# QData/FastSK

Measured on AMD Instinct MI355X. Metric: gkm kernel build: mismatch-combos/s, higher is better.
Workload: dtype u4 count planes (v_dot8_u32_u4), u32 register sums, u64 triangle (plain stores on the first pass over reset rows, else atomics); 1 GPU; config5: synthetic DNA 100000 x 300 bp, g=12 m=8 exact, 495 combos; n_seq=100000, seq_len=300, g=12, m=8, combos=495, parallelism=single GPU

## Files before the change

fastsk_amd/csrc/fsk_engine_dense_shift.hip:

```cpp
#include "fsk_engine_internal.h"
#include "fsk_kernels_dense_shift.h"

#include <map>

using namespace fsk_detail;

namespace fsk {

#define FSK_DMA_SHIFT 1
#define FSK_DMA_KERNEL k_dense_tile_shift
#define FSK_DMA_COMPACT 0
#include "fsk_tile_kernel_dma.inc"
#undef FSK_DMA_KERNEL
#undef FSK_DMA_SHIFT

#define FSK_DMA_SHIFT 2
#define FSK_DMA_KERNEL k_dense_tile_shift_all
#include "fsk_tile_kernel_dma.inc"
#undef FSK_DMA_KERNEL
#undef FSK_DMA_COMPACT
#undef FSK_DMA_SHIFT

}

namespace fsk_detail {

bool dense_shift_plan(fsk_engine* e, const int32_t* combos, int n, u64 by_overflow, uint32_t max_chain) {
    ShiftPlan& p = e->shift;
    if (!(p.by_overflow == by_overflow && p.max_chain == max_chain && (int)p.combos.size() == n && std::equal(combos, combos + n, p.combos.begin()))) {
        p = ShiftPlan();
        p.combos.assign(combos, combos + n);
        p.by_overflow = by_overflow;
        p.max_chain = max_chain;
        const int k = e->k;
        std::map<std::vector<uint8_t>, std::vector<std::pair<int, int>>> shapes;
        for (int q = 0; q < n; ++q) {
            const uint8_t* pos = &e->all_pos[(size_t)combos[q] * k];
            std::vector<uint8_t> shape(pos, pos + k);
            for (auto& x : shape) x = (uint8_t)(x - pos[0]);
            shapes[shape].push_back({(int)pos[0], q});
        }
        std::vector<std::vector<int>> chains;
        for (auto& kv : shapes) {
            auto& v = kv.second;
            std::stable_sort(v.begin(), v.end(), [](const std::pair<int, int>& a, const std::pair<int, int>& b) { return a.first < b.first; });
            for (size_t i = 0; i < v.size(); ++i) {
                if (i == 0 || v[i].first != v[i - 1].first + 1 || (max_chain != 0u && chains.back().size() >= max_chain)) chains.emplace_back();
                chains.back().push_back(v[i].second);
            }
        }
        std::stable_sort(chains.begin(), chains.end(), [](const std::vector<int>& a, const std::vector<int>& b) { return a.size() > b.size(); });
        p.n_bases = (uint32_t)chains.size();
        p.order.resize((size_t)n);
        uint32_t derived = p.n_bases;
        size_t group_begin = 0;
        for (size_t c = 0; c < chains.size(); ++c) {
            const std::vector<int>& ch = chains[c];
            const uint32_t len = (uint32_t)ch.size();
            p.order[c] = ch[0];
            if (c == 0 || chains[c - 1].size() != ch.size() || (u64)(c - group_begin) >= by_overflow) {
                p.groups.push_back(0u);
                p.groups.push_back(len);
                group_begin = c;
            }
            p.groups[p.groups.size() - 2] = (uint32_t)c + 1u;
            uint32_t lower = (uint32_t)c;
            for (uint32_t u = 1; u < len; ++u) {
                const uint32_t upper = derived++;
                p.order[upper] = ch[u];
                p.steps.push_back(upper << 16 | lower);
                p.steps.push_back(len - u);
                p.wsum += len - u;
                lower = upper;
            }
        }
        bool falling = true;
        for (size_t gi = 2; gi + 1 < p.groups.size(); gi += 2) falling = falling && p.groups[gi + 1] < p.groups[gi - 1];
        if (falling) {
            for (size_t gi = 0; gi + 1 < p.groups.size(); gi += 2) {
                p.group_steps.push_back(p.groups[gi]);
                p.group_steps.push_back(p.groups[gi + 1] - (gi + 3 < p.groups.size() ? p.groups[gi + 3] : 0u));
            }
            p.group_steps.push_back(0xffffffffu);
            p.group_steps.push_back(0u);
        }
    }
    return !p.steps.empty() && n <= 32768 && ((u64)2 * e->maxW + 32) * p.wsum < ((u64)1 << 31);
}

int dense_shift_edge_keys(fsk_engine* e, const uint8_t* chunk_pos, uint32_t panels_pad) {
    ShiftPlan& p = e->shift;
    const uint32_t n_steps = (uint32_t)(p.steps.size() / 2), np_seq = panels_pad * fsk::PANEL;
    FSK_HIP(e->d_shift_steps.reserve(p.steps.size() + p.group_steps.size()));
    FSK_HIP(e->d_edge_keys.reserve((size_t)n_steps * np_seq));
    FSK_HIP(hipMemcpyAsync(e->d_shift_steps.p, p.steps.data(), p.steps.size() * sizeof(uint32_t), hipMemcpyHostToDevice, e->stream));
    if (!p.group_steps.empty())
        FSK_HIP(hipMemcpyAsync(e->d_shift_steps.p + p.steps.size(), p.group_steps.data(), p.group_steps.size() * sizeof(uint32_t), hipMemcpyHostToDevice,
                               e->stream));
    FSK_LAUNCH(fsk::k_dense_edge_keys, dim3(panels_pad, (n_steps + 3u) / 4u), dim3(256), 0, e->stream, e->view(), e->cfg.g, e->k, e->sigma, chunk_pos,
               (const uint32_t*)e->d_shift_steps.p, n_steps, np_seq, e->d_edge_keys.p);
    FSK_HIP(hipStreamSynchronize(e->stream));
    e->st.launches += 1;
    return FSK_OK;
}

int dense_shift_keymajor(fsk_engine* e, uint32_t panels_pad, int nb, uint32_t Vq8) {
    const ShiftPlan& p = e->shift;
    e->ld.shift_packed = false;
    if (e->tune.dense_shift_packed < 0 || p.max_chain != SHIFT_PACKED_CHAIN) return FSK_OK;
    const size_t plane = (size_t)panels_pad * Vq8 * fsk::PANEL * (size_t)nb;
    const size_t n_keys = (p.steps.size() / 2) * (size_t)panels_pad * fsk::PANEL;
    const size_t want = (2 * plane + n_keys) * sizeof(uint32_t);
    const char* why = nullptr;
    if (e->tune.dense_shift_plane_kb > 0 && want > (size_t)e->tune.dense_shift_plane_kb * 1024) why = "over the dense_shift_plane_kb cap";
    const size_t grow = (std::max(plane, e->d_KM.cap) - e->d_KM.cap + std::max(plane, e->d_KMH.cap) - e->d_KMH.cap +
                         std::max(n_keys, e->d_edge_offs.cap) - e->d_edge_offs.cap) * sizeof(uint32_t);
    if (!why && grow > 0) {
        size_t free_b = 0, total_b = 0;
        if (hipMemGetInfo(&free_b, &total_b) != hipSuccess) free_b = 0;
        if (grow > free_b / 2) why = "more than half of the free device memory";
        else if (e->d_KM.reserve(plane) != hipSuccess || e->d_KMH.reserve(plane) != hipSuccess || e->d_edge_offs.reserve(n_keys) != hipSuccess) {
            (void)hipGetLastError();
            e->d_KM.release(); e->d_KMH.release(); e->d_edge_offs.release();
            why = "hipMalloc failed";
        }
    }
    if (why) {
        if (e->trace())
            fprintf(stderr, "[fsk] dense shift classes: the key-major planes (%.1f MB) do not fit, %s: k_dense_shift_fix runs the corrections\n",
                    (double)want / 1e6, why);
        return FSK_OK;
    }
    const uint32_t n_pairs = panels_pad / 2u;
    const uint32_t kgrid = (uint32_t)(((size_t)n_pairs * nb * Vq8 * 16u + 255u) / 256u);
    FSK_LAUNCH(fsk::k_dense_keymajor, dim3(kgrid), dim3(256), 0, e->stream, (const uint32_t*)e->d_C4.p, n_pairs, nb, Vq8, e->d_KM.p);
    FSK_LAUNCH(fsk::k_dense_keymajor, dim3(kgrid), dim3(256), 0, e->stream, (const uint32_t*)e->d_C4H.p, n_pairs, nb, Vq8, e->d_KMH.p);
    FSK_LAUNCH(fsk::k_dense_edge_offs, dim3((uint32_t)((n_keys + 255u) / 256u)), dim3(256), 0, e->stream, (const uint16_t*)e->d_edge_keys.p, n_keys,
               e->d_edge_offs.p);
    e->st.launches += 3;
    e->ld.shift_packed = true;
    return FSK_OK;
}

int dense_shift_tiles(fsk_engine* e, u64 n_tiles, int nb, uint32_t Vq8, uint32_t nst, u64* K, int store, uint32_t panels_pad) {
    const ShiftPlan& p = e->shift;
    const bool one_launch = !p.group_steps.empty() && (e->tune.dense_shift_one_launch > 0 ||
                                                       (e->tune.dense_shift_one_launch == 0 && e->tune.tile_splits == 0 && n_tiles >= 16384));
    int base_launches = 1;
    if (one_launch) {
        FSK_LAUNCH(fsk::k_dense_tile_shift_all, dim3((uint32_t)n_tiles, 1), dim3(256), 0, e->stream, (const uint32_t*)e->d_C4.p,
                   (const uint32_t*)e->d_C4H.p, (const uint32_t*)e->d_rowmask.p, (const uint32_t*)e->d_tiletab.p, nb, Vq8, nst, (uint32_t)e->N, K,
                   (int)p.n_bases, store, (const uint32_t*)e->d_shift_steps.p + p.steps.size());
    } else {
        base_launches = (int)(p.groups.size() / 2);
        int slot0 = 0;
        for (size_t gi = 0; gi + 1 < p.groups.size(); gi += 2) {
            const int end = (int)p.groups[gi];
            FSK_LAUNCH(fsk::k_dense_tile_shift, dim3((uint32_t)n_tiles, 1), dim3(256), 0, e->stream, (const uint32_t*)e->d_C4.p,
                       (const uint32_t*)e->d_C4H.p, (const uint32_t*)e->d_rowmask.p, (const uint32_t*)e->d_tiletab.p, nb, Vq8, nst, (uint32_t)e->N, K,
                       end - slot0, gi == 0 ? store : 0, slot0, p.groups[gi + 1]);
            slot0 = end;
        }
    }
    if (e->ld.shift_packed) {
        const auto k_packed = e->tune.dense_shift_inplace != 0 ? fsk::k_dense_shift_packed<true> : fsk::k_dense_shift_packed<false>;
        FSK_LAUNCH(k_packed, dim3((uint32_t)n_tiles), dim3(256), 0, e->stream, (const uint32_t*)e->d_KM.p, (const uint32_t*)e->d_KMH.p,
                   (const uint32_t*)e->d_rowmask.p, (const uint32_t*)e->d_tiletab.p, (const uint32_t*)e->d_shift_steps.p, (uint32_t)(p.steps.size() / 2),
                   (const uint32_t*)e->d_edge_offs.p, panels_pad * fsk::PANEL, nb, Vq8, p.n_bases, (uint32_t)(32u * p.wsum), (uint32_t)e->N, K);
    } else {
        FSK_LAUNCH(fsk::k_dense_shift_fix, dim3((uint32_t)n_tiles), dim3(512), 0, e->stream, (const uint32_t*)e->d_C4.p, (const uint32_t*)e->d_C4H.p,
                   (const uint32_t*)e->d_rowmask.p, (const uint32_t*)e->d_tiletab.p, (const uint32_t*)e->d_shift_steps.p, (uint32_t)(p.steps.size() / 2),
                   (const uint16_t*)e->d_edge_keys.p, panels_pad * fsk::PANEL, nb, Vq8, (uint32_t)e->N, K);
    }
    e->st.launches += (int32_t)base_launches;
    return FSK_OK;
}

}
```

fastsk_amd/csrc/fsk_engine_internal.h:

```cpp
#pragma once
#include "fsk_common.h"

#include <algorithm>
#include <chrono>
#include <cmath>
#include <cstdarg>
#include <cstdio>
#include <cstdlib>
#include <cstring>
#include <string>
#include <array>
#include <atomic>
#include <thread>
#include <vector>

#include <cstdint>
#include <climits>

#include "../../include/fastsk_amd.h"
#include <condition_variable>
#include <functional>
#include <memory>
#include <mutex>

struct fsk_group;

namespace fsk_detail {

#define FSK_HIP(call)                                                                          \
    do {                                                                                       \
        hipError_t _e = (call);                                                                \
        if (_e != hipSuccess) return e->fail(FSK_EDEVICE, "%s failed: %s", #call, hipGetErrorString(_e)); \
    } while (0)

template <typename T>
struct DevBuf {
    T* p = nullptr;
    size_t cap = 0;
    DevBuf() = default;
    DevBuf(DevBuf&& o) noexcept : p(o.p), cap(o.cap) { o.p = nullptr; o.cap = 0; }
    DevBuf& operator=(DevBuf&& o) noexcept { std::swap(p, o.p); std::swap(cap, o.cap); return *this; }
    ~DevBuf() { release(); }
    hipError_t reserve(size_t n) {
        if (n <= cap) return hipSuccess;
        release();
        hipError_t r = hipMalloc((void**)&p, n * sizeof(T));
        if (r == hipSuccess) cap = n;
        return r;
    }
    void release() {
        if (p) (void)hipFree(p);
        p = nullptr;
        cap = 0;
    }
};

template <typename T>
struct PinnedBuf {
    T* p = nullptr;
    size_t cap = 0;
    PinnedBuf() = default;
    PinnedBuf(PinnedBuf&& o) noexcept : p(o.p), cap(o.cap) { o.p = nullptr; o.cap = 0; }
    PinnedBuf& operator=(PinnedBuf&& o) noexcept { std::swap(p, o.p); std::swap(cap, o.cap); return *this; }
    ~PinnedBuf() { release(); }
    hipError_t reserve(size_t n, size_t slack = 0) {
        if (n <= cap) return hipSuccess;
        release();
        hipError_t r = hipHostMalloc((void**)&p, (n + slack) * sizeof(T));
        if (r == hipSuccess) cap = n + slack;
        return r;
    }
    void release() {
        if (p) (void)hipHostFree(p);
        p = nullptr;
        cap = 0;
    }
};

template <typename H, hipError_t (*Create)(H*, unsigned), hipError_t (*Destroy)(H)>
struct Handle {
    H h = nullptr;
    Handle() = default;
    Handle(Handle&& o) noexcept : h(o.h) { o.h = nullptr; }
    Handle& operator=(Handle&& o) noexcept { std::swap(h, o.h); return *this; }
    ~Handle() { if (h) (void)Destroy(h); }
    hipError_t create(unsigned flags) { return h ? hipSuccess : Create(&h, flags); }
    operator H() const { return h; }
};
using Stream = Handle<hipStream_t, hipStreamCreateWithFlags, hipStreamDestroy>;
using Event = Handle<hipEvent_t, hipEventCreateWithFlags, hipEventDestroy>;

struct DeviceScope {
    int prev = -1, dev;
    hipError_t err = hipSuccess;
    explicit DeviceScope(int d) : dev(d) {
        if (hipGetDevice(&prev) != hipSuccess) prev = -1;
        if (prev != dev) err = hipSetDevice(dev);
    }
    ~DeviceScope() {
        if (prev >= 0 && prev != dev) (void)hipSetDevice(prev);
    }
    DeviceScope(const DeviceScope&) = delete;
    DeviceScope& operator=(const DeviceScope&) = delete;
};
#define FSK_ON_DEVICE(e)                                                                      \
    DeviceScope fsk_on_device_((e)->cfg.device);                                             \
    if (fsk_on_device_.err != hipSuccess)                                                    \
        return (e)->fail(FSK_EDEVICE, "hipSetDevice(%d) failed: %s", (e)->cfg.device, hipGetErrorString(fsk_on_device_.err))

}

using fsk_detail::DevBuf;
using fsk_detail::PinnedBuf;
using fsk_detail::Stream;
using fsk_detail::Event;

#define FSK_TUNING_KEYS(X)                                                                                                          \
    X(trace, 0, 0, 1, "stderr: the tuning in force, where the host time of a load and of a variance-mode call goes")                 \
    X(profile, -1, -1, 2, "fsk_config.profile from here on (-1: as the engine was created)")                                          \
    X(compact, -1, -1, 1, "dense: key compaction off / on whatever the alphabet says (-1: a rare symbol decides)")                   \
    X(compact_rare, -1, -1, 1, "dense: keys that occur from the places of the rare symbols (1) or a marking pass over every window (0)") \
    X(tile_splits, 0, 0, 4096, "dense: combo splits per tile (0: by the size of the launch)")                                        \
    X(dense_small, 0, 0, 1, "dense: 1 = a split tile launch (small N) leaves its sums as 32-bit staging blocks that k_dense_widen adds into K (0: one 64-bit atomic a cell and split — measured faster: the atomics drain under other workgroups' dot products)")                                        \
    X(dense_shift, 0, -1, 1, "dense: one weighted Gram product per chain of shifted combinations, the other members by edge lookups (fsk_engine_dense_shift.hip) — 1 = whenever the call is eligible, -1 = never (0: when eligible, tile_splits = 0 and the launch has 16384 tiles or more, the size from which a tile has one workgroup anyway)") \
    X(dense_shift_packed, 0, -1, 0, "dense, shift classes: the derived steps from key-major planes, eight cells an LDS read (k_dense_keymajor, k_dense_shift_packed; chains cut at nine members) — 0 = whenever the shift path runs and the planes fit, -1 = never: k_dense_shift_fix on the count panels") \
    X(dense_shift_inplace, 1, 0, 1, "dense, shift classes: k_dense_shift_packed stages a chain's first planes and makes every further step's in LDS, one nibble up and one down a sequence (a step that meets a count above 15 in its tile, and the step behind it, are staged) — 0 = every step staged") \
    X(dense_shift_one_launch, 0, -1, 1, "dense, shift classes: every chain-length group of the base products in ONE launch that flushes at the group ends without clearing (k_dense_tile_shift_all) — 1 = whenever the shift path runs, -1 = never: one k_dense_tile_shift launch a group (0: where the shift path runs by its own default rule, tile_splits = 0 and 16384 tiles or more)") \
    X(dense_shift_plane_kb, 0, 0, (int64_t)1 << 40, "dense, shift classes: the key-major planes and offsets may take this many KiB at most (0: half of the free memory; tests: the planes do not fit)") \
    X(dense_chunk, 0, 0, 1 << 24, "dense: cap of the count kernel's staging chunk, in windows (0: none)")                             \
    X(variance_dense_slots, 1, 0, 1, "variance mode, dense: 0 = zero fill + k_welford per iteration instead of storing slot triangles") \
    X(var_slots16, 1, 0, 1, "variance mode, sparse: 0 = u32 slot triangles from the start")                                          \
    X(sparse_global, 0, 0, 1, "sparse: every += as a 64-bit atomicAdd (k_sx_emit<DIRECT>) whatever N is")                             \
    X(sparse_unpacked, 0, 0, 1, "sparse: entries in the general 8 + 4 (+ 4) byte format whatever N is")                               \
    X(sparse_pairs, 1, 0, 1, "sparse: 0 = every update word 32 bits wide (1: unit products of clean runs travel two to a word)")      \
    X(sparse_sync, 0, 0, 1, "sparse: wait for every batch's word count and size its stream exactly")                                 \
    X(sparse_hint, 1, 0, 1, "sparse: 0 = the words per record of the previous set of sequences are never kept as a hint")             \
    X(sparse_exact_lanes, 0, 0, 2, "sparse: the batches of an exact accumulate never (1) / always (2) in two lanes (0: from six batches on)") \
    X(sparse_batch_records, 0, 0, (int64_t)1 << 31, "sparse: records per batch at most (0: 2^27)")                                   \
    X(guard_cap, 0, 0, (int64_t)1 << 40, "sparse: pretend the stream buffer holds this many words (0: its real size)")                \
    X(list_max_words, 0, 0, (int64_t)1 << 31, "sparse: update words of one batch beyond which its pairs go to K with atomics (0: 2^31)") \
    X(seg_scan_chunked, 0, 0, 1, "sparse: the three-launch segment scan whatever the tile count")                                    \
    X(extract_slots, 0, 0, 4, "sparse: slots per k_sx_extract_win workgroup, 1 or 4 (0: by the size of the launch)")                  \
    X(sparse_form, 0, 0, 3, "sparse: the update stage — 1 = owner bands whenever they exist, 2 = two-level blocks, 3 = 64-bit atomics (0: bands up to four LDS rounds a band, blocks beyond)") \
    X(blocks_sub_shift, 14, 4, 14, "sparse, blocks: log2 of the cells one k_sxb_consume workgroup sums in LDS (tests: small blocks on small inputs)") \
    X(blocks_max_bands, 512, 2, 512, "sparse, blocks: bands of one pass at most (tests: several passes on small inputs)")            \
    X(blocks_band_shift_max, 23, 4, 23, "sparse, blocks: log2 of a band's cells at most (tests)")                                    \
    X(blocks_pass_words, 0, 0, (int64_t)1 << 32, "sparse, blocks: update words of one pass at most (0: 2^31)")                       \
    X(sparse_desc, 0, -1, 1, "sparse, owner bands and two-level blocks: entries of many partners leave k_sx_emit as descriptors (one an entry; blocks: one per sub-band its partners fall into) that k_sx_consume / k_sxb_consume expand in LDS — 1 = always, -1 = never (0: once a batch of these sequences has shown sparse_desc_from pairs per record)") \
    X(sparse_desc_blocks, 1, 0, 1, "sparse, two-level blocks: 0 = never descriptors there (1: as sparse_desc says — one record per sub-band an entry's partners fall into)") \
    X(sparse_desc_cols, 1, 0, 3, "sparse, descriptors: where the partners are read from — 0 = the entries themselves; 1 = a column array (sequence id | multiplicity, 4 bytes) beside 8-byte entries, the entries themselves when they are packed (measured: 2-byte columns beside packed entries are no faster, 0.88 against 0.84 s in the large-g regime; 4-byte columns beside 8-byte entries 4.69 -> 4.44 ms a combo at N = 100k); tests: 2 = 4-byte columns always, 3 = 2-byte columns when N < 32768") \
    X(sparse_desc_min, 16, 1, 48, "sparse, descriptors: entries of more partners than this become descriptors (48: everything k_sx_emit does not bin in LDS; measured, large-g regime: 48 0.92 s, 32 0.85, 16 0.83-0.85, 8 0.88, 4 0.90)") \
    X(sparse_desc_from, 12, 1, 1 << 20, "sparse, descriptors: the pairs per sort record of a batch from which on the following batches use them (sparse_desc = 0)") \
    X(sparse_parts_target, 0, 0, 1 << 30, "sparse, owner bands: words of one k_sx_consume part (0: four LDS rounds' worth at least, 1/1024 of the batch's words; tests: several parts a band on small inputs)") \
    X(sparse_desc_parts, 2048, 1, 1 << 16, "sparse, descriptors: parts (k_sx_consume workgroups) the bands' streams are cut into, about") \
    X(sparse_share, 0, -1, 254, "sparse: leading kept positions sorted once per group of consecutive combos that share them (0: by cost; -1: never); batches of more than 16 slots only (smaller ones read their positions by id), and never when the presort's scratch passes a quarter of the free memory") \
    X(seed_splitmix, 0, 0, 1, "approx modes: 1 = fsk_set_seed draws the engine's older splitmix64 Fisher-Yates order (0: the reference's std::shuffle of minstd_rand0)") \
    X(mismatch_order, 0, 0, 1, "mismatch-weighted mode: 1 = the levels run from m = d down to 0 (0: from 0 up to d)")                   \
    X(collective, 0, 0, 2, "fsk_create_multi: FSK_COLL_* when fsk_config.collective is FSK_COLL_AUTO")                                \
    X(deadline_ms, 120000, -1, 86400000, "fsk_create_multi: the fail-fast bound when fsk_config.deadline_ms is 0 (negative: none)")   \
    X(svm_wg_max, 8192, 0, 8192, "fsk_svm_train: up to this many training rows the solver is one workgroup with alpha, G and y in LDS (k_svm_wg); beyond, two launches an iteration (k_svm_select_i / k_svm_select_j); 0 = always those") \
    X(svm_chunk, 256, 1, 65536, "fsk_svm_train: iterations enqueued between two reads of the solver's status record (k_svm_wg: iterations a launch)") \
    X(rows_tile, FSK_ROWS_TILE, FSK_ROWS_TILE, FSK_ROWS_TILE, "fsk_rows_build, read-only: the edge T of k_rows_syrk's tile of the rows kernel (compiled in)") \
    X(rows_panel, FSK_ROWS_PANEL, FSK_ROWS_PANEL, FSK_ROWS_PANEL, "fsk_rows_build, read-only: the consecutive train columns P a panel of k_rows_syrk stages in LDS (compiled in)") \
    FSK_TUNING_TEST_KEYS(X)
#ifdef FSK_TEST_HOOKS
#define FSK_TUNING_TEST_KEYS(X)                                            \
    X(fault_kind, 0, 0, 3, "test hook: 1 = host sleep, 2 = device spin before a band's collective; 3 = host sleep after the variance chains")   \
    X(fault_rank, -1, -1, 15, "test hook: the engine that is late")        \
    X(fault_band, -1, -1, 63, "test hook: before this band's collective")  \
    X(fault_ms, 0, 0, 60000, "test hook: by this many milliseconds")
#else
#define FSK_TUNING_TEST_KEYS(X)
#endif
struct fsk_tuning {
#define FSK_X(name, def, lo, hi, doc) int64_t name = (def);
    FSK_TUNING_KEYS(FSK_X)
#undef FSK_X
};

struct SxScratch {
    DevBuf<unsigned char> d_keys[2];
    DevBuf<uint32_t> d_blockhist, d_totals, d_tile_ent, d_ebase, d_Pk, d_Tk, d_ucount, d_uchunk, d_utot, d_list_off, d_ulist, d_part_base;
    DevBuf<u64> d_tile_stat;
    DevBuf<uint32_t> d_segc;
    DevBuf<int> d_tile_lrh, d_tile_rs, d_tile_lth, d_tile_ts;
    DevBuf<uint2> d_E;
    DevBuf<u64> d_sxstat;
    DevBuf<uint32_t> d_group_of, d_group_head, d_winp;
    DevBuf<unsigned char> d_part;
    DevBuf<uint32_t> d_ulist2, d_subcnt, d_suboff, d_subcur;
    DevBuf<uint32_t> d_dsubcnt, d_dsuboff, d_dsubcur;
    DevBuf<uint32_t> d_cols;
};

struct ShiftPlan {
    std::vector<int32_t> combos;
    u64 by_overflow = 0;
    std::vector<int32_t> order;
    std::vector<uint32_t> groups, steps, group_steps;
    uint32_t n_bases = 0;
    uint32_t max_chain = 0;
    u64 wsum = 0;
};

struct SvmCvState {
    bool valid = false;
    std::vector<double> oof;
    std::vector<fsk_svm_cv_score> scores;
    std::vector<fsk_svm_cv_problem> problems;
    std::vector<double> alpha;
    std::vector<uint32_t> idx;
    std::vector<u64> st_off, idx_off;
    fsk_svm_cv_info info{};
    DevBuf<double> d_alpha, d_G, d_krow, d_coef, d_rho, d_oof;
    DevBuf<uint32_t> d_idx;
    DevBuf<int32_t> d_fold;
    DevBuf<signed char> d_y;
    DevBuf<unsigned char> d_prob, d_rec;
};

struct SvmState {
    bool valid = false;
    SvmCvState cv;
    std::vector<double> alpha;
    std::vector<signed char> y;
    double rho = 0;
    int kernel = 0;
    double w_pos = 1.0, w_neg = 1.0;
    double C = 0, eps = 0;
    int64_t max_iter = 0;
    SvmCvState cal;
    bool platt_valid = false;
    fsk_svm_platt_info platt{};
    fsk_svm_info info{};
    DevBuf<double> d_alpha, d_G, d_krow, d_coef, d_out;
    DevBuf<signed char> d_y;
    DevBuf<unsigned char> d_rec;
};

struct RowsState {
    bool valid = false;
    DevBuf<double> d_L, d_diag;
    fsk_rows_info info{};
    void drop() { valid = false; d_L.release(); d_diag.release(); }
};

struct fsk_engine {
    Stream stream;
    Stream lane_stream;
    Stream chain_stream;
    fsk_config cfg{};
    int cfg_profile0 = 0;
    fsk_tuning tune{};
    std::string err;
    int k = 0;
    int64_t ncomb = 0;
    Event ev0, ev1;
    Event ev_out, ev_in;
    fsk_group* group = nullptr;
    bool store_next = false;
    PinnedBuf<uint32_t> h_stage;
    bool stage_in_flight = false;
    PinnedBuf<double> h_prod;

    struct Loaded {
        bool featseq_ready = false;
        bool rare_ready = false;
        bool prep_valid = false, prep_overflow = false, prep_shift = false, shift_packed = false;
        uint32_t prep_chain = 0;
        double vc_sum = 0, vc_n = 0;
        bool u_known = false, u_pending = false;
        u64 u_value = 0, u_extra = 0;
        struct SxDefer { bool active = false; u64 cap = 0, nrec = 0; } sx_defer[8];
        int64_t lazy_lo = -1, lazy_hi = -1;
        std::vector<double> stdevs;
        u64 sx_passes = 0;
        int sx_form_used = -1;
        bool sx_desc_used = false;
        int sx_share_used = 0;
// ... 273 lines not shown
```

fastsk_amd/csrc/fsk_kernels_dense_shift.h:

```cpp
#pragma once
#include "fsk_bytesel.h"
#include "fsk_common.h"

namespace fsk {

__device__ __forceinline__ uint32_t panel_seq(uint32_t p) { return (p >> 2) + 16u * (p & 3u); }

__global__ __launch_bounds__(256) void k_dense_edge_keys(SeqView S, int g, int k, uint32_t sigma, const uint8_t* combo_pos, const uint32_t* steps,
                                                         uint32_t n_steps, uint32_t np_seq, uint16_t* keys) {
    const uint32_t r = threadIdx.x & 63u, step = blockIdx.y * 4u + (threadIdx.x >> 6), panel = blockIdx.x;
    if (step >= n_steps) return;
    const uint32_t seq = panel * PANEL + r;
    const uint32_t sl = steps[2u * step], up = sl >> 16, lo = sl & 0xffffu;
    uint32_t kd = 0, ks = 0;
    if (seq < S.n_seq) {
        const uint32_t len = S.len[seq], wbase = S.wstart[seq];
        if (len >= (uint32_t)g) {
            const uint32_t last = len - (uint32_t)g;
            for (int c = 0; c < k; ++c) {
                kd = kd * sigma + fetch_sym(S.words, wbase, (uint32_t)combo_pos[(size_t)lo * k + c], S.bits);
                ks = ks * sigma + fetch_sym(S.words, wbase, last + (uint32_t)combo_pos[(size_t)up * k + c], S.bits);
            }
        }
    }
// ... 18 lines not shown
    int accR[2][QW], accC[2][QW];
#pragma unroll
    for (int h = 0; h < 2; ++h)
#pragma unroll
        for (int q = 0; q < QW; ++q) accR[h][q] = accC[h][q] = 0;

    const fsk_hw::lds_addr_t lds_wave = fsk_hw::lds_address(P) + w * 1024u;
    auto load_stage = [&](const uint32_t* plane, int buf, uint32_t sl) {
        const uint32_t up = sl >> 16, lo = sl & 0xffffu;
#pragma unroll
        for (int q = 0; q < 4; ++q) {
            const uint32_t panel = (q < 2 ? ti : tj) * 2u + (uint32_t)(q & 1);
            const uint32_t* src = plane + panel * panel_stride + (size_t)(q < 2 ? up : lo) * slot_stride;
            fsk_hw::panel_rows_to_lds(src, Vq8 * PANEL * 4u, lds_wave + (uint32_t)(buf * PBUF + q * HALF) * 4u, tid * 16u);
        }
    };
    auto load_meta = [&](uint32_t s, uint32_t sl, uint32_t& kA, uint32_t& kB, uint32_t& fl) {
        const uint16_t* ks = keys + (size_t)s * np_seq;
        kA = (uint32_t)ks[ti * TILE + lane] | (uint32_t)ks[ti * TILE + PANEL + lane] << 16;
        kB = (uint32_t)ks[tj * TILE + lane] | (uint32_t)ks[tj * TILE + PANEL + lane] << 16;
        const uint32_t up = sl >> 16, lo = sl & 0xffffu;
        const uint32_t mA = rowmask[(size_t)(ti * 2u) * n_slots + up] | rowmask[(size_t)(ti * 2u + 1u) * n_slots + up];
        const uint32_t mB = rowmask[(size_t)(tj * 2u) * n_slots + lo] | rowmask[(size_t)(tj * 2u + 1u) * n_slots + lo];
        fl = mA | mB;
    };
    auto edge = [&](const uint32_t* p0, size_t stride, uint32_t kk, int mul, int& a0, int& a1) {
        const uint32_t kd = kk & 255u, ks = (kk >> 8) & 255u;
        const uint32_t* rd = p0 + (kd >> 3) * PANEL + lane;
        const uint32_t* rs = p0 + (ks >> 3) * PANEL + lane;
        const uint32_t shd = (kd & 7u) * 4u, shs = (ks & 7u) * 4u;
        a0 += ((int)((rs[0] >> shs) & 15u) - (int)((rd[0] >> shd) & 15u)) * mul;
        a1 += ((int)((rs[stride] >> shs) & 15u) - (int)((rd[stride] >> shd) & 15u)) * mul;
    };

    uint32_t sl_cur = steps[0], wt_cur = steps[1];
    uint32_t sl_nxt = n_steps > 1u ? steps[2] : 0u, wt_nxt = n_steps > 1u ? steps[3] : 0u;
    uint32_t kA_n, kB_n, fl_n;
    load_meta(0u, sl_cur, kA_n, kB_n, fl_n);
    uint32_t sl_n2 = 0u, wt_n2 = 0u;
    int buf = 0;
    load_stage(C4, 0, (uint32_t)__builtin_amdgcn_readfirstlane(fsk_hw::vgpr_copy(sl_cur)));
    fsk_hw::wait_panel_rows();
    __syncthreads();
    const uint32_t lsel = (w & 3u) * (uint32_t)QW, hsh = (w >> 2) * 16u;
    for (uint32_t s = 0; s < n_steps; ++s) {
        const uint32_t kA = fsk_hw::vgpr_copy(kA_n), kB = fsk_hw::vgpr_copy(kB_n);
        const uint32_t fl = (uint32_t)__builtin_amdgcn_readfirstlane(fsk_hw::vgpr_copy(fl_n));
        const uint32_t sl = (uint32_t)__builtin_amdgcn_readfirstlane(fsk_hw::vgpr_copy(sl_cur));
        const int wt = (int)((uint32_t)__builtin_amdgcn_readfirstlane(fsk_hw::vgpr_copy(wt_cur)) & 255u);
        if (s + 1u < n_steps) {
            const uint32_t sn = (uint32_t)__builtin_amdgcn_readfirstlane(fsk_hw::vgpr_copy(sl_nxt));
            if (s + 2u < n_steps) {
                sl_n2 = steps[2u * (s + 2u)];
                wt_n2 = steps[2u * (s + 2u) + 1u];
            }
            load_meta(s + 1u, sn, kA_n, kB_n, fl_n);
            load_stage(C4, buf ^ 1, sn);
        }
        const uint32_t* pb = P + buf * PBUF;
        auto lookups = [&](int mul) {
#pragma unroll
            for (int q = 0; q < QW; ++q) {
                const uint32_t kk = (fsk_hw::readlane(kB, lsel + (uint32_t)q) >> hsh) & 0xffffu;
                edge(pb, (size_t)HALF, kk, mul, accR[0][q], accR[1][q]);
                if ((q & 3) == 3) asm volatile("" ::: "memory");
            }
#pragma unroll
            for (int q = 0; q < QW; ++q) {
                const uint32_t kk = (fsk_hw::readlane(kA, lsel + (uint32_t)q) >> hsh) & 0xffffu;
                edge(pb + 2 * HALF, (size_t)HALF, kk, mul, accC[0][q], accC[1][q]);
                if ((q & 3) == 3) asm volatile("" ::: "memory");
            }
        };
        lookups(wt);
        if (fl != 0u) {
            __syncthreads();
            load_stage(C4H, buf, sl);
            fsk_hw::wait_panel_rows();
            __syncthreads();
            lookups(16 * wt);
        }
        fsk_hw::wait_panel_rows();
        __syncthreads();
        sl_cur = sl_nxt; wt_cur = wt_nxt;
        sl_nxt = sl_n2; wt_nxt = wt_n2;
        buf ^= 1;
    }
    int* const T = reinterpret_cast<int*>(P);
#pragma unroll
    for (int h = 0; h < 2; ++h)
#pragma unroll
        for (int q = 0; q < QW; ++q) {
            const uint32_t i = (uint32_t)h * PANEL + lane, j = w * (uint32_t)QW + (uint32_t)q;
            T[i * TILE + ((j + i) & (TILE - 1u))] = accR[h][q];
        }
    __syncthreads();
#pragma unroll
    for (int h = 0; h < 2; ++h) {
        const uint32_t jd = (uint32_t)h * PANEL + lane;
        const u64 j = (u64)tj * TILE + (uint32_t)h * PANEL + panel_seq(lane);
#pragma unroll
        for (int q = 0; q < QW; ++q) {
            const uint32_t id = w * (uint32_t)QW + (uint32_t)q;
            const u64 i = (u64)ti * TILE + (id >> 6) * PANEL + panel_seq(id & 63u);
            const int v = accC[h][q] + T[id * TILE + ((jd + id) & (TILE - 1u))];
            if (i < N && j <= i && v != 0) atomicAdd(&K[tri_index(i, j)], (u64)(long long)v);
        }
    }
}

__device__ __forceinline__ uint32_t km_swizzle(uint32_t key) { return ((key >> 1) & 3u) << 2; }
__device__ __forceinline__ uint32_t km_offset(uint32_t key) { return key << 6 | km_swizzle(key) << 2; }

__global__ __launch_bounds__(256) void k_dense_keymajor(const uint32_t* plane, uint32_t n_pairs, int n_slots, uint32_t Vq8, uint32_t* KM) {
    const size_t id = (size_t)blockIdx.x * 256u + threadIdx.x;
    const uint32_t t = (uint32_t)id & 15u;
    size_t rest = id >> 4;
    const uint32_t row = (uint32_t)(rest % Vq8);
    rest /= Vq8;
    const uint32_t slot = (uint32_t)(rest % (uint32_t)n_slots);
    const size_t pair = rest / (uint32_t)n_slots;
    if (pair >= n_pairs) return;
    const size_t slot_stride = (size_t)Vq8 * PANEL, panel_stride = (size_t)n_slots * slot_stride;
    const uint32_t* src = plane + 2u * pair * panel_stride + slot * slot_stride + (size_t)row * PANEL + 4u * t;
    const uint4 a = *reinterpret_cast<const uint4*>(src), b = *reinterpret_cast<const uint4*>(src + panel_stride);
    const uint32_t in[8] = {a.x, a.y, a.z, a.w, b.x, b.y, b.z, b.w};
    uint32_t* out = KM + (pair * (size_t)n_slots + slot) * ((size_t)Vq8 * 128u);
#pragma unroll
    for (uint32_t q = 0; q < 8u; ++q) {
        uint32_t v = 0;
#pragma unroll
        for (uint32_t n = 0; n < 8u; ++n) v |= ((in[n] >> (4u * q)) & 15u) << (4u * n);
        const uint32_t key = row * 8u + q;
        out[key * 16u + (t ^ km_swizzle(key))] = v;
    }
}

__global__ __launch_bounds__(256) void k_dense_edge_offs(const uint16_t* keys, size_t n, uint32_t* offs) {
    const size_t q = (size_t)blockIdx.x * 256u + threadIdx.x;
    if (q >= n) return;
    const uint32_t kk = keys[q];
    offs[q] = km_offset(kk & 255u) | km_offset(kk >> 8) << 16;
}

template <bool INPLACE>
__global__ __launch_bounds__(256, 2) void k_dense_shift_packed(const uint32_t* KM, const uint32_t* KMH, const uint32_t* rowmask, const uint32_t* tile_tab,
                                                               const uint32_t* steps, uint32_t n_steps, const uint32_t* offs, uint32_t np_seq,
                                                               int n_slots, uint32_t Vq8, uint32_t n_bases, uint32_t bias, uint32_t N, u64* K) {
    constexpr uint32_t SIDE = 256u * 16u;
    constexpr uint32_t PBUF = 2u * SIDE;
    __shared__ __attribute__((aligned(1024))) uint32_t P[2 * PBUF];
    const uint32_t tid = threadIdx.x, lane = tid & 63u;
    const uint32_t w = (uint32_t)__builtin_amdgcn_readfirstlane(tid >> 6);
    const uint32_t M4 = (uint32_t)__builtin_amdgcn_readfirstlane(fsk_hw::vgpr_copy(0x0f0f0f0fu)), B4 = fsk_hw::vgpr_copy(0x10101010u);
    const uint32_t tr = (w >> 1) * 8u + (lane >> 3), tc = (w & 1u) * 8u + (lane & 7u);
    const uint32_t tile = tile_tab[blockIdx.x];
    const uint32_t ti = tile >> 16, tj = tile & 0xffffu;
    const size_t slot_stride = (size_t)Vq8 * 128u;
    const size_t pair_stride = (size_t)n_slots * slot_stride;
    const uint32_t side_bytes = Vq8 * 512u;

    uint32_t acc[8][8], Rr[2][8], Rc[2][8];
#pragma unroll
    for (int a = 0; a < 8; ++a) {
#pragma unroll
        for (int b = 0; b < 8; ++b) acc[a][b] = 0u;
        Rr[0][a] = Rr[1][a] = Rc[0][a] = Rc[1][a] = 0u;
    }

    const fsk_hw::lds_addr_t lds_wave = fsk_hw::lds_address(P) + w * 1024u;
    auto load_stage = [&](const uint32_t* plane, uint32_t buf, uint32_t sl) {
        const uint32_t up = sl >> 16, lo = sl & 0xffffu;
#pragma unroll
        for (uint32_t side = 0; side < 2u; ++side) {
            const uint32_t* src = plane + (side == 0u ? ti : tj) * pair_stride + (size_t)(side == 0u ? up : lo) * slot_stride;
#pragma unroll
            for (uint32_t q = 0; q < 4u; ++q)
                if (q * 4096u < side_bytes)
                    fsk_hw::panel_rows_to_lds(src, side_bytes, lds_wave + (buf * PBUF + side * SIDE + q * 1024u) * 4u, q * 4096u + tid * 16u);
        }
    };
    auto load_offs = [&](uint32_t s, uint4 (&oR)[2], uint4 (&oC)[2]) {
        const uint32_t* os = offs + (size_t)s * np_seq;
#pragma unroll
        for (uint32_t h = 0; h < 2u; ++h) {
            oR[h] = *reinterpret_cast<const uint4*>(os + ti * TILE + h * PANEL + 4u * tr);
            oC[h] = *reinterpret_cast<const uint4*>(os + tj * TILE + h * PANEL + 4u * tc);
        }
    };
    auto flagged = [&](uint32_t sl) {
        const uint32_t up = sl >> 16, lo = sl & 0xffffu;
        const uint32_t mA = rowmask[(size_t)(ti * 2u) * n_slots + up] | rowmask[(size_t)(ti * 2u + 1u) * n_slots + up];
        const uint32_t mB = rowmask[(size_t)(tj * 2u) * n_slots + lo] | rowmask[(size_t)(tj * 2u + 1u) * n_slots + lo];
        return mA | mB;
    };
    auto lds_at = [&](uint32_t byte_off) { return *reinterpret_cast<const uint32_t*>(reinterpret_cast<const char*>(P) + byte_off); };

    uint32_t sl = steps[0], wt = steps[1] & 255u, fl = flagged(sl);
    uint32_t sn = n_steps > 1u ? steps[2] : 0u, wn = n_steps > 1u ? steps[3] : 0u;
    uint32_t s2 = 0u, w2 = 0u, fl_nx = 0u;
    if constexpr (INPLACE) {
        if (n_steps > 2u) { s2 = steps[4]; w2 = steps[5]; }
        if (n_steps > 1u) fl_nx = flagged(sn);
    }
    uint4 oR_n[2], oC_n[2];
    load_offs(0u, oR_n, oC_n);
    uint32_t buf = 0;
    load_stage(KM, 0u, sl);
    fsk_hw::wait_panel_rows();
    __syncthreads();
    for (uint32_t s = 0; s < n_steps; ++s) {
        uint32_t oR[8], oC[8];
#pragma unroll
        for (int h = 0; h < 2; ++h) {
            oR[4 * h] = fsk_hw::vgpr_copy(oR_n[h].x); oR[4 * h + 1] = fsk_hw::vgpr_copy(oR_n[h].y);
            oR[4 * h + 2] = fsk_hw::vgpr_copy(oR_n[h].z); oR[4 * h + 3] = fsk_hw::vgpr_copy(oR_n[h].w);
            oC[4 * h] = fsk_hw::vgpr_copy(oC_n[h].x); oC[4 * h + 1] = fsk_hw::vgpr_copy(oC_n[h].y);
            oC[4 * h + 2] = fsk_hw::vgpr_copy(oC_n[h].z); oC[4 * h + 3] = fsk_hw::vgpr_copy(oC_n[h].w);
        }
        const bool same = INPLACE && s + 1u < n_steps && (sn & 0xffffu) >= n_bases && fl == 0u && fl_nx == 0u;
        uint32_t uo_n = 0u;
        if (s + 1u < n_steps) {
            load_offs(s + 1u, oR_n, oC_n);
            if (same) uo_n = offs[(size_t)(w < 2u ? s + 1u : s) * np_seq + (w < 2u ? ti : tj) * TILE + (tid & 127u)];
            else load_stage(KM, buf ^ 1u, sn);
        }
        if ((sl & 0xffffu) < n_bases) {
#pragma unroll
            for (int a = 0; a < 8; ++a) Rr[0][a] = Rr[1][a] = Rc[0][a] = Rc[1][a] = 0u;
        }
        const uint32_t baseA = buf * PBUF * 4u, baseB = baseA + SIDE * 4u;
        const uint32_t xA = (tr * 4u) | baseA, xB = (tc * 4u) | baseB;
        uint32_t dA[8], sA[8], dB[8], sB[8];
        auto read_A = [&](int e) { dA[e] = lds_at(fsk_hw::xor_word<0>(oC[e], xA)); sA[e] = lds_at(fsk_hw::xor_word<1>(oC[e], xA)); };
        auto read_B = [&](int e) { dB[e] = lds_at(fsk_hw::xor_word<0>(oR[e], xB)); sB[e] = lds_at(fsk_hw::xor_word<1>(oR[e], xB)); };
        auto row_term = [&](int e) {
            Rr[0][e] += ((sA[e] & M4) | B4) - (dA[e] & M4);
            Rr[1][e] += (((sA[e] >> 4) & M4) | B4) - ((dA[e] >> 4) & M4);
            acc[0][e] = fsk_hw::add_byte<0>(acc[0][e], Rr[0][e]); acc[1][e] = fsk_hw::add_byte<0>(acc[1][e], Rr[1][e]);
            acc[2][e] = fsk_hw::add_byte<1>(acc[2][e], Rr[0][e]); acc[3][e] = fsk_hw::add_byte<1>(acc[3][e], Rr[1][e]);
            acc[4][e] = fsk_hw::add_byte<2>(acc[4][e], Rr[0][e]); acc[5][e] = fsk_hw::add_byte<2>(acc[5][e], Rr[1][e]);
            acc[6][e] = fsk_hw::add_byte<3>(acc[6][e], Rr[0][e]); acc[7][e] = fsk_hw::add_byte<3>(acc[7][e], Rr[1][e]);
        };
        auto col_term = [&](int e) {
            Rc[0][e] += ((sB[e] & M4) | B4) - (dB[e] & M4);
            Rc[1][e] += (((sB[e] >> 4) & M4) | B4) - ((dB[e] >> 4) & M4);
            acc[e][0] = fsk_hw::add_byte<0>(acc[e][0], Rc[0][e]); acc[e][1] = fsk_hw::add_byte<0>(acc[e][1], Rc[1][e]);
            acc[e][2] = fsk_hw::add_byte<1>(acc[e][2], Rc[0][e]); acc[e][3] = fsk_hw::add_byte<1>(acc[e][3], Rc[1][e]);
            acc[e][4] = fsk_hw::add_byte<2>(acc[e][4], Rc[0][e]); acc[e][5] = fsk_hw::add_byte<2>(acc[e][5], Rc[1][e]);
            acc[e][6] = fsk_hw::add_byte<3>(acc[e][6], Rc[0][e]); acc[e][7] = fsk_hw::add_byte<3>(acc[e][7], Rc[1][e]);
        };
#pragma unroll
        for (int e = 0; e < 8; ++e) read_A(e);
        fsk_hw::first_use(dA[0], sA[0], dA[1], sA[1], dA[2], sA[2], dA[3], sA[3]);
#pragma unroll
        for (int e = 0; e < 4; ++e) read_B(e);
#pragma unroll
        for (int e = 0; e < 4; ++e) row_term(e);
        fsk_hw::first_use(dA[4], sA[4], dA[5], sA[5], dA[6], sA[6], dA[7], sA[7]);
#pragma unroll
        for (int e = 4; e < 8; ++e) read_B(e);
#pragma unroll
        for (int e = 4; e < 8; ++e) row_term(e);
        fsk_hw::first_use(dB[0], sB[0], dB[1], sB[1], dB[2], sB[2], dB[3], sB[3]);
#pragma unroll
        for (int e = 0; e < 4; ++e) col_term(e);
        fsk_hw::first_use(dB[4], sB[4], dB[5], sB[5], dB[6], sB[6], dB[7], sB[7]);
#pragma unroll
        for (int e = 4; e < 8; ++e) col_term(e);
        if (fl != 0u) {
            __syncthreads();
            load_stage(KMH, buf, sl);
            fsk_hw::wait_panel_rows();
            __syncthreads();
            const uint32_t mul = 16u * wt;
#pragma unroll
            for (int e = 0; e < 8; ++e) {
                read_A(e);
                read_B(e);
#pragma unroll
                for (int n = 0; n < 8; ++n) {
                    acc[n][e] += (((sA[e] >> (4 * n)) & 15u) - ((dA[e] >> (4 * n)) & 15u)) * mul;
                    acc[e][n] += (((sB[e] >> (4 * n)) & 15u) - ((dB[e] >> (4 * n)) & 15u)) * mul;
                }
            }
        }
        uint32_t fl_n = 0u, sl_n2 = 0u, wt_n2 = 0u;
        if constexpr (INPLACE) {
            if (s + 2u < n_steps) {
                fl_n = flagged(s2);
                if (s + 3u < n_steps) {
                    sl_n2 = steps[2u * (s + 3u)];
                    wt_n2 = steps[2u * (s + 3u) + 1u];
                }
            }
        } else if (s + 1u < n_steps) {
            fl_n = flagged(sn);
            if (s + 2u < n_steps) {
                sl_n2 = steps[2u * (s + 2u)];
                wt_n2 = steps[2u * (s + 2u) + 1u];
            }
        }
        fsk_hw::wait_panel_rows();
        __syncthreads();
        if (same) {
            const uint32_t uo = fsk_hw::vgpr_copy(uo_n), od = uo & 0xffffu, os = uo >> 16;
            if (od != os) {
                const uint32_t p = tid & 127u, t4 = p & 0x3cu, e = (p >> 6) * 4u + (p & 3u);
                const uint32_t base = buf * PBUF + (w >> 1) * SIDE, inc = 1u << (4u * e);
                atomicAdd(&P[base + ((os ^ t4) >> 2)], inc);
                atomicAdd(&P[base + ((od ^ t4) >> 2)], 0u - inc);
            }
            __syncthreads();
        } else {
            buf ^= 1u;
        }
        if constexpr (INPLACE) {
            sl = sn; wt = wn & 255u; fl = fl_nx;
            sn = s2; wn = w2; fl_nx = fl_n;
            s2 = sl_n2; w2 = wt_n2;
        } else {
            sl = sn; wt = wn & 255u; fl = fl_n;
            sn = sl_n2; wn = wt_n2;
        }
    }
#pragma unroll
    for (int er = 0; er < 8; ++er) {
        const u64 i = (u64)ti * TILE + tile_index(tr, (uint32_t)er);
#pragma unroll
        for (int ec = 0; ec < 8; ++ec) {
            const u64 j = (u64)tj * TILE + tile_index(tc, (uint32_t)ec);
            const int v = (int)(acc[er][ec] - bias);
            if (i < N && j <= i && v != 0) atomicAdd(&K[tri_index(i, j)], (u64)(long long)v);
        }
    }
}

}
```

Measured before the change: 453.0 combos/s.

## Batch per-step prefix sums in byte accumulators before flushing into int32 sums

In k_dense_shift_packed, each step no longer scatters its row and column running sums into the 8x8 accumulator grid with add_byte. It now adds them into byte-packed second-level sums (Qr/Qc) and flushes those into acc only when the step table's flag bit 256 is set. The host computes these flags so that a batch never overflows a byte, charging 30(r+1) per step at chain position r against 255. The bias trick is also changed from OR-ing 0x10 per nibble to adding ~d & 0xf, which makes the per-step bias 15 instead of 16, so the bias argument drops from 32*wsum to 30*wsum. This cuts the many add_byte operations per step at the cost of extra registers (Qr/Qc) and a flag-driven branch, which may reduce occupancy.

```diff
diff --git a/fastsk_amd/csrc/fsk_engine_dense_shift.hip b/fastsk_amd/csrc/fsk_engine_dense_shift.hip
--- a/fastsk_amd/csrc/fsk_engine_dense_shift.hip
+++ b/fastsk_amd/csrc/fsk_engine_dense_shift.hip
@@ -88,12 +88,29 @@
     return !p.steps.empty() && n <= 32768 && ((u64)2 * e->maxW + 32) * p.wsum < ((u64)1 << 31);
 }
 
+static void dense_shift_unpack_flags(std::vector<uint32_t>& steps, uint32_t n_bases, bool batch) {
+    const size_t n_steps = steps.size() / 2;
+    uint32_t r = 0, bound = 0;
+    for (size_t s = 0; s < n_steps; ++s) {
+        r = (steps[2 * s] & 0xffffu) < n_bases ? 0u : r + 1u;
+        const uint32_t add = 30u * (r + 1u);
+        if (s > 0 && (!batch || bound + add > 255u)) {
+            steps[2 * s - 1] |= 256u;
+            bound = 0;
+        }
+        bound += add;
+    }
+    if (n_steps > 0) steps[2 * n_steps - 1] |= 256u;
+}
+
 int dense_shift_edge_keys(fsk_engine* e, const uint8_t* chunk_pos, uint32_t panels_pad) {
     ShiftPlan& p = e->shift;
     const uint32_t n_steps = (uint32_t)(p.steps.size() / 2), np_seq = panels_pad * fsk::PANEL;
+    std::vector<uint32_t> steps = p.steps;
+    dense_shift_unpack_flags(steps, p.n_bases, e->tune.dense_shift_batch != 0);
     FSK_HIP(e->d_shift_steps.reserve(p.steps.size() + p.group_steps.size()));
     FSK_HIP(e->d_edge_keys.reserve((size_t)n_steps * np_seq));
-    FSK_HIP(hipMemcpyAsync(e->d_shift_steps.p, p.steps.data(), p.steps.size() * sizeof(uint32_t), hipMemcpyHostToDevice, e->stream));
+    FSK_HIP(hipMemcpyAsync(e->d_shift_steps.p, steps.data(), steps.size() * sizeof(uint32_t), hipMemcpyHostToDevice, e->stream));
     if (!p.group_steps.empty())
         FSK_HIP(hipMemcpyAsync(e->d_shift_steps.p + p.steps.size(), p.group_steps.data(), p.group_steps.size() * sizeof(uint32_t), hipMemcpyHostToDevice,
                                e->stream));
@@ -166,7 +183,7 @@
         const auto k_packed = e->tune.dense_shift_inplace != 0 ? fsk::k_dense_shift_packed<true> : fsk::k_dense_shift_packed<false>;
         FSK_LAUNCH(k_packed, dim3((uint32_t)n_tiles), dim3(256), 0, e->stream, (const uint32_t*)e->d_KM.p, (const uint32_t*)e->d_KMH.p,
                    (const uint32_t*)e->d_rowmask.p, (const uint32_t*)e->d_tiletab.p, (const uint32_t*)e->d_shift_steps.p, (uint32_t)(p.steps.size() / 2),
-                   (const uint32_t*)e->d_edge_offs.p, panels_pad * fsk::PANEL, nb, Vq8, p.n_bases, (uint32_t)(32u * p.wsum), (uint32_t)e->N, K);
+                   (const uint32_t*)e->d_edge_offs.p, panels_pad * fsk::PANEL, nb, Vq8, p.n_bases, (uint32_t)(30u * p.wsum), (uint32_t)e->N, K);
     } else {
         FSK_LAUNCH(fsk::k_dense_shift_fix, dim3((uint32_t)n_tiles), dim3(512), 0, e->stream, (const uint32_t*)e->d_C4.p, (const uint32_t*)e->d_C4H.p,
                    (const uint32_t*)e->d_rowmask.p, (const uint32_t*)e->d_tiletab.p, (const uint32_t*)e->d_shift_steps.p, (uint32_t)(p.steps.size() / 2),
diff --git a/fastsk_amd/csrc/fsk_engine_internal.h b/fastsk_amd/csrc/fsk_engine_internal.h
--- a/fastsk_amd/csrc/fsk_engine_internal.h
+++ b/fastsk_amd/csrc/fsk_engine_internal.h
@@ -125,6 +125,7 @@
     X(dense_shift, 0, -1, 1, "dense: one weighted Gram product per chain of shifted combinations, the other members by edge lookups (fsk_engine_dense_shift.hip) — 1 = whenever the call is eligible, -1 = never (0: when eligible, tile_splits = 0 and the launch has 16384 tiles or more, the size from which a tile has one workgroup anyway)") \
     X(dense_shift_packed, 0, -1, 0, "dense, shift classes: the derived steps from key-major planes, eight cells an LDS read (k_dense_keymajor, k_dense_shift_packed; chains cut at nine members) — 0 = whenever the shift path runs and the planes fit, -1 = never: k_dense_shift_fix on the count panels") \
     X(dense_shift_inplace, 1, 0, 1, "dense, shift classes: k_dense_shift_packed stages a chain's first planes and makes every further step's in LDS, one nibble up and one down a sequence (a step that meets a count above 15 in its tile, and the step behind it, are staged) — 0 = every step staged") \
+    X(dense_shift_batch, 1, 0, 1, "dense, shift classes: k_dense_shift_packed adds the prefix sums of several steps byte to byte and hands the bytes to its int32 sums once a batch, where the step table says so (a step at chain position r counts 30 (r + 1) against a byte's 255; a batch may span chains) — 0 = after every step") \
     X(dense_shift_one_launch, 0, -1, 1, "dense, shift classes: every chain-length group of the base products in ONE launch that flushes at the group ends without clearing (k_dense_tile_shift_all) — 1 = whenever the shift path runs, -1 = never: one k_dense_tile_shift launch a group (0: where the shift path runs by its own default rule, tile_splits = 0 and 16384 tiles or more)") \
     X(dense_shift_plane_kb, 0, 0, (int64_t)1 << 40, "dense, shift classes: the key-major planes and offsets may take this many KiB at most (0: half of the free memory; tests: the planes do not fit)") \
     X(dense_chunk, 0, 0, 1 << 24, "dense: cap of the count kernel's staging chunk, in windows (0: none)")                             \
diff --git a/fastsk_amd/csrc/fsk_kernels_dense_shift.h b/fastsk_amd/csrc/fsk_kernels_dense_shift.h
--- a/fastsk_amd/csrc/fsk_kernels_dense_shift.h
+++ b/fastsk_amd/csrc/fsk_kernels_dense_shift.h
@@ -194,7 +194,7 @@
     __shared__ __attribute__((aligned(1024))) uint32_t P[2 * PBUF];
     const uint32_t tid = threadIdx.x, lane = tid & 63u;
     const uint32_t w = (uint32_t)__builtin_amdgcn_readfirstlane(tid >> 6);
-    const uint32_t M4 = (uint32_t)__builtin_amdgcn_readfirstlane(fsk_hw::vgpr_copy(0x0f0f0f0fu)), B4 = fsk_hw::vgpr_copy(0x10101010u);
+    const uint32_t M4 = (uint32_t)__builtin_amdgcn_readfirstlane(fsk_hw::vgpr_copy(0x0f0f0f0fu));
     const uint32_t tr = (w >> 1) * 8u + (lane >> 3), tc = (w & 1u) * 8u + (lane & 7u);
     const uint32_t tile = tile_tab[blockIdx.x];
     const uint32_t ti = tile >> 16, tj = tile & 0xffffu;
@@ -202,12 +202,13 @@
     const size_t pair_stride = (size_t)n_slots * slot_stride;
     const uint32_t side_bytes = Vq8 * 512u;
 
-    uint32_t acc[8][8], Rr[2][8], Rc[2][8];
+    uint32_t acc[8][8], Rr[2][8], Rc[2][8], Qr[2][8], Qc[2][8];
 #pragma unroll
     for (int a = 0; a < 8; ++a) {
 #pragma unroll
         for (int b = 0; b < 8; ++b) acc[a][b] = 0u;
         Rr[0][a] = Rr[1][a] = Rc[0][a] = Rc[1][a] = 0u;
+        Qr[0][a] = Qr[1][a] = Qc[0][a] = Qc[1][a] = 0u;
     }
 
     const fsk_hw::lds_addr_t lds_wave = fsk_hw::lds_address(P) + w * 1024u;
@@ -238,7 +239,7 @@
     };
     auto lds_at = [&](uint32_t byte_off) { return *reinterpret_cast<const uint32_t*>(reinterpret_cast<const char*>(P) + byte_off); };
 
-    uint32_t sl = steps[0], wt = steps[1] & 255u, fl = flagged(sl);
+    uint32_t sl = steps[0], wt = steps[1], fl = flagged(sl);
     uint32_t sn = n_steps > 1u ? steps[2] : 0u, wn = n_steps > 1u ? steps[3] : 0u;
     uint32_t s2 = 0u, w2 = 0u, fl_nx = 0u;
     if constexpr (INPLACE) {
@@ -277,20 +278,16 @@
         auto read_A = [&](int e) { dA[e] = lds_at(fsk_hw::xor_word<0>(oC[e], xA)); sA[e] = lds_at(fsk_hw::xor_word<1>(oC[e], xA)); };
         auto read_B = [&](int e) { dB[e] = lds_at(fsk_hw::xor_word<0>(oR[e], xB)); sB[e] = lds_at(fsk_hw::xor_word<1>(oR[e], xB)); };
         auto row_term = [&](int e) {
-            Rr[0][e] += ((sA[e] & M4) | B4) - (dA[e] & M4);
-            Rr[1][e] += (((sA[e] >> 4) & M4) | B4) - ((dA[e] >> 4) & M4);
-            acc[0][e] = fsk_hw::add_byte<0>(acc[0][e], Rr[0][e]); acc[1][e] = fsk_hw::add_byte<0>(acc[1][e], Rr[1][e]);
-            acc[2][e] = fsk_hw::add_byte<1>(acc[2][e], Rr[0][e]); acc[3][e] = fsk_hw::add_byte<1>(acc[3][e], Rr[1][e]);
-            acc[4][e] = fsk_hw::add_byte<2>(acc[4][e], Rr[0][e]); acc[5][e] = fsk_hw::add_byte<2>(acc[5][e], Rr[1][e]);
-            acc[6][e] = fsk_hw::add_byte<3>(acc[6][e], Rr[0][e]); acc[7][e] = fsk_hw::add_byte<3>(acc[7][e], Rr[1][e]);
+            Rr[0][e] += (sA[e] & M4) + (~dA[e] & M4);
+            Rr[1][e] += ((sA[e] >> 4) & M4) + (~(dA[e] >> 4) & M4);
+            Qr[0][e] += Rr[0][e];
+            Qr[1][e] += Rr[1][e];
         };
         auto col_term = [&](int e) {
-            Rc[0][e] += ((sB[e] & M4) | B4) - (dB[e] & M4);
-            Rc[1][e] += (((sB[e] >> 4) & M4) | B4) - ((dB[e] >> 4) & M4);
-            acc[e][0] = fsk_hw::add_byte<0>(acc[e][0], Rc[0][e]); acc[e][1] = fsk_hw::add_byte<0>(acc[e][1], Rc[1][e]);
-            acc[e][2] = fsk_hw::add_byte<1>(acc[e][2], Rc[0][e]); acc[e][3] = fsk_hw::add_byte<1>(acc[e][3], Rc[1][e]);
-            acc[e][4] = fsk_hw::add_byte<2>(acc[e][4], Rc[0][e]); acc[e][5] = fsk_hw::add_byte<2>(acc[e][5], Rc[1][e]);
-            acc[e][6] = fsk_hw::add_byte<3>(acc[e][6], Rc[0][e]); acc[e][7] = fsk_hw::add_byte<3>(acc[e][7], Rc[1][e]);
+            Rc[0][e] += (sB[e] & M4) + (~dB[e] & M4);
+            Rc[1][e] += ((sB[e] >> 4) & M4) + (~(dB[e] >> 4) & M4);
+            Qc[0][e] += Rc[0][e];
+            Qc[1][e] += Rc[1][e];
         };
 #pragma unroll
         for (int e = 0; e < 8; ++e) read_A(e);
@@ -310,12 +307,29 @@
         fsk_hw::first_use(dB[4], sB[4], dB[5], sB[5], dB[6], sB[6], dB[7], sB[7]);
 #pragma unroll
         for (int e = 4; e < 8; ++e) col_term(e);
+        if ((wt & 256u) != 0u) {
+#pragma unroll
+            for (int e = 0; e < 8; ++e) {
+                acc[0][e] = fsk_hw::add_byte<0>(acc[0][e], Qr[0][e]); acc[1][e] = fsk_hw::add_byte<0>(acc[1][e], Qr[1][e]);
+                acc[2][e] = fsk_hw::add_byte<1>(acc[2][e], Qr[0][e]); acc[3][e] = fsk_hw::add_byte<1>(acc[3][e], Qr[1][e]);
+                acc[4][e] = fsk_hw::add_byte<2>(acc[4][e], Qr[0][e]); acc[5][e] = fsk_hw::add_byte<2>(acc[5][e], Qr[1][e]);
+                acc[6][e] = fsk_hw::add_byte<3>(acc[6][e], Qr[0][e]); acc[7][e] = fsk_hw::add_byte<3>(acc[7][e], Qr[1][e]);
+            }
+#pragma unroll
+            for (int e = 0; e < 8; ++e) {
+                acc[e][0] = fsk_hw::add_byte<0>(acc[e][0], Qc[0][e]); acc[e][1] = fsk_hw::add_byte<0>(acc[e][1], Qc[1][e]);
+                acc[e][2] = fsk_hw::add_byte<1>(acc[e][2], Qc[0][e]); acc[e][3] = fsk_hw::add_byte<1>(acc[e][3], Qc[1][e]);
+                acc[e][4] = fsk_hw::add_byte<2>(acc[e][4], Qc[0][e]); acc[e][5] = fsk_hw::add_byte<2>(acc[e][5], Qc[1][e]);
+                acc[e][6] = fsk_hw::add_byte<3>(acc[e][6], Qc[0][e]); acc[e][7] = fsk_hw::add_byte<3>(acc[e][7], Qc[1][e]);
+                Qr[0][e] = Qr[1][e] = Qc[0][e] = Qc[1][e] = 0u;
+            }
+        }
         if (fl != 0u) {
             __syncthreads();
             load_stage(KMH, buf, sl);
             fsk_hw::wait_panel_rows();
             __syncthreads();
-            const uint32_t mul = 16u * wt;
+            const uint32_t mul = 16u * (wt & 255u);
 #pragma unroll
             for (int e = 0; e < 8; ++e) {
                 read_A(e);
@@ -358,11 +372,11 @@
             buf ^= 1u;
         }
         if constexpr (INPLACE) {
-            sl = sn; wt = wn & 255u; fl = fl_nx;
+            sl = sn; wt = wn; fl = fl_nx;
             sn = s2; wn = w2; fl_nx = fl_n;
             s2 = sl_n2; w2 = wt_n2;
         } else {
-            sl = sn; wt = wn & 255u; fl = fl_n;
+            sl = sn; wt = wn; fl = fl_n;
             sn = sl_n2; wn = wt_n2;
         }
     }
```

Measured after the change: 464.5 combos/s (median of 6 runs). 2.5% higher.
